# Corv/CUDA-GMM-MPI

Measured on NVIDIA H100. Metric: EM iterations/sec at N=10M D=24 K=64; E-step HBM GB/s vs roofline, higher is better.
Workload: dtype f32

## Files before the change

### cuda-gmm-mpi_b200/csrc/kernels_tc.cu

```cuda
#include <cuda.h>
#include <cudaTypedefs.h>
#include <cuda_fp16.h>
#if defined(__F16C__) && defined(__AVX__)
#include <immintrin.h>
#endif
#include <cuda_runtime.h>

#include <cfloat>
#include <cmath>
#include <cstdio>
#include <cstdlib>
#include <cstring>
#include <string>
#include <type_traits>
#include <vector>

#include "host_math.h"
#include "kernels_tc.cuh"
#include "mstep_rows.h"
#include "tc_ptx.cuh"

namespace gmm {

using namespace ptx;

#define TC_CUDA_TRY(expr)                                                                     \
    do {                                                                                      \
        cudaError_t e_ = (expr);                                                              \
        if (e_ != cudaSuccess)                                                                \
            return fail(GMM_ERR_CUDA, std::string(#expr) + ": " + cudaGetErrorString(e_));    \
    } while (0)

constexpr int kTE = 32;
constexpr int kNCL = 32;
constexpr int kNST = 3;
constexpr int kNRAW = 4;
constexpr int kChunkSub = 4;
constexpr int kChunkSub2 = 16;
constexpr int kPhiBits = 11;
constexpr float kGammaScale = 1024.0f;
constexpr float kGammaMagic = 1.5f * 134217728.0f;

template <int D, int NCL_> struct MCfg {
    static_assert(D % 4 == 0, "tensor M-step: D must be a multiple of 4");
    static_assert(NCL_ == 32 || NCL_ == 64, "tensor M-step: 32 or 64 clusters per CTA");
    static constexpr int NCL = NCL_;
    static constexpr int HPC = 64 / NCL;
    static constexpr int F = 1 + D + D * (D + 1) / 2;
    static constexpr int S = D / 4;
    static constexpr int MT = (4 * ((1 + 2 * S + S * (D / 2) + 7) / 8) * 8 + 127) / 128;
    static constexpr int G_PART = NCL * kTE * 2;
    static constexpr int G_STAGE = 3 * G_PART;
    static constexpr int RAWZ = (D * kTE * 4 + 1023) / 1024 * 1024;
    static constexpr int RAWX = RAWZ + 1024;
    static constexpr int RAWG = NCL * kTE * 4;
    static constexpr int OFF_G = 0;
    static constexpr int OFF_RAWX = OFF_G + kNST * G_STAGE;
    static constexpr int OFF_RAWG = OFF_RAWX + kNRAW * RAWX;
    static constexpr int NCT = MT * 128;
    static constexpr int OFF_RACC = OFF_RAWG + kNRAW * RAWG;
    static constexpr int OFF_BAR = OFF_RACC + 32 * NCT * 4;
    static constexpr int SMEM_BYTES = OFF_BAR + 512;
    static constexpr int THREADS = 128 + NCT;
    static constexpr int REG_LAUNCH = (65536 / THREADS) / 8 * 8 > 255 ? 255 : (65536 / THREADS) / 8 * 8;
    static constexpr int REG_P = MT == 1 ? REG_LAUNCH : 56;
    static constexpr int REG_C = MT == 3 ? 152 : (MT == 2 ? 224 : REG_LAUNCH);
    static_assert(128 * REG_P + NCT * REG_C <= THREADS * REG_LAUNCH, "register pools");
    static_assert(OFF_RAWX % 1024 == 0 && RAWX % 1024 == 0 && RAWZ % 1024 == 0, "SWIZZLE_128B TMA destinations need 1024-byte alignment");
    static_assert(OFF_RAWG % 1024 == 0 && RAWG % 1024 == 0, "SWIZZLE_128B TMA destinations need 1024-byte alignment");
    static_assert(MT <= 3, "feature tiles");
};

template <int R, int L>
__device__ __forceinline__ void set_regs() {
    if constexpr (R < L) asm volatile("setmaxnreg.dec.sync.aligned.u32 %0;" ::"n"(R));
    else if constexpr (R > L) asm volatile("setmaxnreg.inc.sync.aligned.u32 %0;" ::"n"(R));
}

struct MMagic { float lin, prod; };

__device__ __forceinline__ void tma_load_2d(void* smem_dst, const CUtensorMap* tmap, int c0, int c1, uint64_t* bar) {
    asm volatile(
        "cp.async.bulk.tensor.2d.shared::cluster.global.mbarrier::complete_tx::bytes [%0], [%1, {%2, %3}], [%4];"
        ::"r"(smem_u32(smem_dst)), "l"(reinterpret_cast<uint64_t>(tmap)), "r"(c0), "r"(c1), "r"(smem_u32(bar)) : "memory");
}

__device__ __forceinline__ float2 lds_f2(uint32_t addr) {
    float2 v;
    asm volatile("ld.shared.v2.f32 {%0, %1}, [%2];" : "=f"(v.x), "=f"(v.y) : "r"(addr) : "memory");
    return v;
}

__device__ __forceinline__ void feature_split(float a, float b, float m, float& h, float& l) {
    h = __fsub_rn(__fmaf_rn(a, b, m), m);
    l = __fmaf_rn(a, b, -h);
}

#ifndef GMM_MSTEP_CUT
#define GMM_MSTEP_CUT 0
#endif

__device__ __forceinline__ void build_half(const float2 (&za)[4], const float2 (&zb0)[4], const float2 (&zb1)[4], float m0, float m1,
                                           uint32_t (&hi)[2][4], uint32_t (&lo)[2][4]) {
#pragma unroll
    for (int p = 0; p < 4; p++) {
        const int ks = p >> 1, u = p & 1;
#if GMM_MSTEP_CUT == 2
        hi[ks][2 * u] = __float_as_uint(zb0[p].x); hi[ks][2 * u + 1] = __float_as_uint(zb1[p].x);
        lo[ks][2 * u] = __float_as_uint(zb0[p].y); lo[ks][2 * u + 1] = __float_as_uint(zb1[p].y);
        (void)za; (void)m0; (void)m1;
#else
        float h0, l0, h1, l1, h2, l2, h3, l3;
        feature_split(za[p].x, zb0[p].x, m0, h0, l0);
        feature_split(za[p].y, zb0[p].y, m0, h1, l1);
        feature_split(za[p].x, zb1[p].x, m1, h2, l2);
        feature_split(za[p].y, zb1[p].y, m1, h3, l3);
        hi[ks][2 * u] = pack_half2(h0, h1);
        hi[ks][2 * u + 1] = pack_half2(h2, h3);
        lo[ks][2 * u] = pack_half2(l0, l1);
        lo[ks][2 * u + 1] = pack_half2(l2, l3);
#endif
    }
}

__device__ __forceinline__ void load_row(uint32_t addr, float2 (&z)[4]) {
#pragma unroll
    for (int p = 0; p < 4; p++) z[p] = lds_f2(addr ^ (uint32_t)(p << 5));
}

template <int NCL>
__device__ __forceinline__ void issue_half(float (&ex)[NCL / 2], float (&rm)[NCL / 2], const uint32_t (&hi)[2][4], const uint32_t (&lo)[2][4],
                                           uint32_t gam, bool new1, bool new2) {
#pragma unroll
    for (int ks = 0; ks < kTE / 16; ks++) {
        const uint64_t hdesc = make_smem_desc(gam + ks * 256,  128,  512);
        const uint64_t ldesc = make_smem_desc(gam + NCL * kTE * 2 + ks * 256, 128, 512);
        const uint64_t sdesc = make_smem_desc(gam + 2 * NCL * kTE * 2 + ks * 256, 128, 512);
#if GMM_MSTEP_CUT == 1
        asm volatile("" ::"r"(hi[ks][0]), "r"(hi[ks][1]), "r"(hi[ks][2]), "r"(hi[ks][3]), "r"(lo[ks][0]), "r"(lo[ks][1]), "r"(lo[ks][2]),
                     "r"(lo[ks][3]), "l"(hdesc), "l"(ldesc), "l"(sdesc));
        (void)ex; (void)rm; (void)new1; (void)new2;
#else
        if constexpr (NCL == 32) {
            wgmma_m64n32k16_rs(ex, hi[ks][0], hi[ks][1], hi[ks][2], hi[ks][3], hdesc, ks > 0 || !new1);
            wgmma_m64n32k16_rs(rm, hi[ks][0], hi[ks][1], hi[ks][2], hi[ks][3], ldesc, ks > 0 || !new2);
            wgmma_m64n32k16_rs(rm, lo[ks][0], lo[ks][1], lo[ks][2], lo[ks][3], sdesc, true);
        } else {
            wgmma_m64n64k16_rs(ex, hi[ks][0], hi[ks][1], hi[ks][2], hi[ks][3], hdesc, ks > 0 || !new1);
            wgmma_m64n64k16_rs(rm, hi[ks][0], hi[ks][1], hi[ks][2], hi[ks][3], ldesc, ks > 0 || !new2);
            wgmma_m64n64k16_rs(rm, lo[ks][0], lo[ks][1], lo[ks][2], lo[ks][3], sdesc, true);
        }
#endif
    }
}

__device__ __forceinline__ bool chain_ends(int i, int mt, int nsub) { return ((i + mt) % kChunkSub) == kChunkSub - 1 || i == nsub - 1; }
__device__ __forceinline__ bool chain_starts(int i, int mt) { return i == 0 || ((i + mt) % kChunkSub) == 0; }
__device__ __forceinline__ bool chain2_ends(int i, int mt, int nsub) { return ((i + mt) % kChunkSub2) == kChunkSub2 - 1 || i == nsub - 1; }
__device__ __forceinline__ bool chain2_starts(int i, int mt) { return i == 0 || ((i + mt) % kChunkSub2) == 0; }

template <int D, int NCL, bool WT = false>
__global__ void __launch_bounds__(MCfg<D, NCL>::THREADS, 1)
mstep_tc_kernel(const __grid_constant__ CUtensorMap tm_x, const __grid_constant__ CUtensorMap tm_g, int n, int K,
                float* __restrict__ scratch, int events_per_cta, const __grid_constant__ MMagic magic, const int* __restrict__ opmap,
                const float* __restrict__ wts, float w_max, float w_inv) {
    using C = MCfg<D, NCL>;
    constexpr int HPC = C::HPC;
    extern __shared__ __align__(1024) uint8_t smem[];
    uint64_t* bars = reinterpret_cast<uint64_t*>(smem + C::OFF_BAR);
    uint64_t* raw_full = bars;
    uint64_t* raw_empty = bars + kNRAW;
    uint64_t* op_full = bars + 2 * kNRAW;
    uint64_t* op_empty = op_full + kNST;

    const int warp = threadIdx.x >> 5, lane = threadIdx.x & 31;
    const int range = blockIdx.x / (2 / HPC), part = blockIdx.x % (2 / HPC);
    const int e_begin = range * events_per_cta;
    const int e_end = min(n, e_begin + events_per_cta);
    const int nsub = (e_end - e_begin + kTE - 1) / kTE;
    const int k0 = blockIdx.y * NCL;

    for (int i = threadIdx.x; i < kNRAW * 256; i += C::THREADS)
        reinterpret_cast<float*>(smem + C::OFF_RAWX + (i >> 8) * C::RAWX + C::RAWZ)[i & 255] = 1.0f;
    if (threadIdx.x == 0) {
        for (int s = 0; s < kNRAW; s++) { mbar_init(&raw_full[s], 1); mbar_init(&raw_empty[s], 3 + 4 * C::MT); }
        for (int s = 0; s < kNST; s++) { mbar_init(&op_full[s], 3); mbar_init(&op_empty[s], 4 * C::MT); }
        fence_mbar_init();
    }
    __syncthreads();

    if (warp < 4) {
        set_regs<C::REG_P, C::REG_LAUNCH>();
        if (warp == 0) {
            const int nbox = min(NCL, K - k0 + kNCL - 1) / kNCL;
            if (elect_one()) {
                for (int i = 0; i < nsub; i++) {
                    const int st = i % kNRAW, ph = (i / kNRAW) & 1;
                    mbar_wait_parked(&raw_empty[st], ph ^ 1, 500);
                    mbar_arrive_expect_tx(&raw_full[st], kTE * D * 4 + nbox * kNCL * kTE * 4);
                    const int e0 = e_begin + i * kTE;
                    tma_load_2d(smem + C::OFF_RAWX + st * C::RAWX, &tm_x, e0, 0, &raw_full[st]);
                    for (int b = 0; b < nbox; b++)
                        tma_load_2d(smem + C::OFF_RAWG + st * C::RAWG + b * kNCL * kTE * 4, &tm_g, e0, k0 + b * kNCL, &raw_full[st]);
                }
            }
        } else {
            const int bt = threadIdx.x - 32;
            constexpr int NITEM = 4 * NCL, NIT = (NITEM + 95) / 96;
            for (int i = 0; i < nsub; i++) {
                const int rs = i % kNRAW, rph = (i / kNRAW) & 1;
                const int os = i % kNST, oph = (i / kNST) & 1;
                [[maybe_unused]] float wv[8];
                if constexpr (WT) {
                    const float4* wp = reinterpret_cast<const float4*>(wts + e_begin + i * kTE + 8 * ((bt & 31) >> 3));
                    const float4 wa = __ldg(wp), wb = __ldg(wp + 1);
                    wv[0] = wa.x; wv[1] = wa.y; wv[2] = wa.z; wv[3] = wa.w; wv[4] = wb.x; wv[5] = wb.y; wv[6] = wb.z; wv[7] = wb.w;
#pragma unroll
                    for (int v = 0; v < 8; v++) wv[v] = wv[v] == w_max ? 1.0f : __fmul_rn(wv[v], w_inv);
                }
                mbar_wait_parked(&raw_full[rs], rph, 200);
                mbar_wait_parked(&op_empty[os], oph ^ 1, 200);
                uint8_t* g_hi = smem + C::OFF_G + os * C::G_STAGE;
                float dep = 0.0f;
#pragma unroll
                for (int u = 0; u < NIT; u++) {
                    const int it = bt + 96 * u;
                    if (it >= NITEM) break;
                    const int kg = it >> 5, l = it & 31;
                    const int k = kg * 8 + (l & 7), ce = l >> 3;
                    const uint8_t* grow = smem + C::OFF_RAWG + rs * C::RAWG + k * (kTE * 4);
                    const float4 a = *reinterpret_cast<const float4*>(grow + (((2 * ce) ^ (k & 7)) << 4));
                    const float4 b = *reinterpret_cast<const float4*>(grow + (((2 * ce + 1) ^ (k & 7)) << 4));
                    float g[8] = {a.x, a.y, a.z, a.w, b.x, b.y, b.z, b.w};
                    dep += a.x + b.x;
                    if constexpr (WT) {
#pragma unroll
                        for (int v = 0; v < 8; v++) g[v] = __fmul_rn(g[v], wv[v]);
                    }
                    float hi[8], lo[8];
#pragma unroll
                    for (int v = 0; v < 8; v++) {
                        hi[v] = __fsub_rn(__fmaf_rn(g[v], kGammaScale, kGammaMagic), kGammaMagic);
                        lo[v] = __fmaf_rn(g[v], kGammaScale, -hi[v]);
                    }
                    *reinterpret_cast<uint4*>(g_hi + kg * 512 + l * 16) =
                        make_uint4(pack_half2(hi[0], hi[1]), pack_half2(hi[2], hi[3]), pack_half2(hi[4], hi[5]), pack_half2(hi[6], hi[7]));
                    *reinterpret_cast<uint4*>(g_hi + C::G_PART + kg * 512 + l * 16) =
                        make_uint4(pack_half2(lo[0], lo[1]), pack_half2(lo[2], lo[3]), pack_half2(lo[4], lo[5]), pack_half2(lo[6], lo[7]));
                    *reinterpret_cast<uint4*>(g_hi + 2 * C::G_PART + kg * 512 + l * 16) =
                        make_uint4(pack_half2(g[0] * kGammaScale, g[1] * kGammaScale), pack_half2(g[2] * kGammaScale, g[3] * kGammaScale),
                                   pack_half2(g[4] * kGammaScale, g[5] * kGammaScale), pack_half2(g[6] * kGammaScale, g[7] * kGammaScale));
                }
                __syncwarp();
                if (lane == 0) mbar_arrive_after(&raw_empty[rs], dep);
                else asm volatile("" ::"f"(dep));
                fence_proxy_async_smem();
                __syncwarp();
                if (lane == 0) mbar_arrive(&op_full[os]);
            }
        }
    } else {
        set_regs<C::REG_C, C::REG_LAUNCH>();
        const int cw = __shfl_sync(0xffffffffu, (warp - 4) >> 2, 0);
        const int hx = HPC == 2 ? 2 * cw : part * C::MT + cw;
        const int mt = hx >> 1;
        const int ct = threadIdx.x - 128;
        const int wq = warp & 3, gid = lane >> 2, qd = lane & 3;
        float* racc = reinterpret_cast<float*>(smem + C::OFF_RACC) + ct;
#pragma unroll
        for (int j = 0; j < 32; j++) racc[j * C::NCT] = 0.0f;
        constexpr int NSLOT = 2 * HPC;
        uint32_t fa, fb[NSLOT];
        float mg[NSLOT];
        {
            const int* om = opmap + hx * 64 + wq * 16 + gid;
            auto addr = [&](int code) {
                const uint32_t row = code >= kRowOne ? (uint32_t)(C::RAWZ / 128 + code - kRowOne) : (uint32_t)code;
                return row * 128 + ((((uint32_t)qd >> 1) ^ (row & 7)) << 4) + ((uint32_t)qd & 1) * 8;
            };
#pragma unroll
            for (int s = 0; s < NSLOT; s++) {
                const int c = om[(s >> 1) * 64 + (s & 1) * 8];
                const int a = c & 255, b = c >> 8;
                if (s == 0) fa = addr(a);
                fb[s] = addr(b);
                mg[s] = a >= kRowOne && b >= kRowOne ? 0.0f : (a >= kRowOne || b >= kRowOne ? magic.lin : magic.prod);
            }
        }
        const uint32_t zs0 = smem_u32(smem + C::OFF_RAWX);
        float ex[HPC][NCL / 2], rm[HPC][NCL / 2];
#pragma unroll
        for (int h = 0; h < HPC; h++)
#pragma unroll
            for (int j = 0; j < NCL / 2; j++) { ex[h][j] = 0.0f; rm[h][j] = 0.0f; }
        auto add_to_racc = [&](float (&acc)[HPC][NCL / 2]) {
#pragma unroll
            for (int c = 0; c < 2; c++) {
#pragma unroll
                for (int j = 0; j < 16; j++) {
                    const int q = 16 * c + j;
                    racc[q * C::NCT] += acc[q / (NCL / 2)][q % (NCL / 2)];
                }
                asm volatile("" ::: "memory");
            }
        };
        uint32_t fh[2][2][4], fl[2][2][4];
        float2 za[4];
        int held = -1;
        auto group = [&](int i, auto hc, uint32_t (&gh)[2][4], uint32_t (&gl)[2][4]) {
            constexpr int h = decltype(hc)::value;
            const int rs = i % kNRAW, rph = (i / kNRAW) & 1;
            const int os = i % kNST, oph = (i / kNST) & 1;
            const uint32_t zst = zs0 + rs * C::RAWX;
            const uint32_t gam = smem_u32(smem + C::OFF_G + os * C::G_STAGE);
            const bool new1 = chain_starts(i, mt), new2 = chain2_starts(i, mt);
            if constexpr (h == 0) {
                mbar_wait_parked(&raw_full[rs], rph, 100);
                load_row(zst + fa, za);
            }
            float2 zb0[4], zb1[4];
            load_row(zst + fb[2 * h], zb0);
            load_row(zst + fb[2 * h + 1], zb1);
            build_half(za, zb0, zb1, mg[2 * h], mg[2 * h + 1], gh, gl);
            if constexpr (h == 0) mbar_wait_parked(&op_full[os], oph, 100);
            wgmma_fence();
            issue_half<NCL>(ex[h], rm[h], gh, gl, gam, new1, new2);
            wgmma_commit();
            if constexpr (h == HPC - 1) {
                __syncwarp();
                if (lane == 0) mbar_arrive(&raw_empty[rs]);
            }
            wgmma_wait<1>();
            if constexpr (h == 0) {
                __syncwarp();
                if (lane == 0 && held >= 0) mbar_arrive(&op_empty[held]);
            }
            if constexpr (h == HPC - 1) {
                held = os;
                if (chain_ends(i, mt, nsub)) {
                    wgmma_wait<0>();
                    __syncwarp();
                    if (lane == 0) mbar_arrive(&op_empty[os]);
                    held = -1;
#if GMM_MSTEP_CUT != 3
                    add_to_racc(ex);
                    if (chain2_ends(i, mt, nsub)) add_to_racc(rm);
#endif
                }
            }
        };
        using H0 = std::integral_constant<int, 0>;
        using H1 = std::integral_constant<int, 1>;
        if constexpr (HPC == 2) {
            for (int i = 0; i < nsub; i++) {
                group(i, H0{}, fh[0], fl[0]);
                group(i, H1{}, fh[1], fl[1]);
            }
        } else {
            int i = 0;
            for (; i + 1 < nsub; i += 2) {
                group(i, H0{}, fh[0], fl[0]);
                group(i + 1, H0{}, fh[1], fl[1]);
            }
            if (i < nsub) group(i, H0{}, fh[0], fl[0]);
        }
        wgmma_wait<0>();
#if GMM_MSTEP_CUT == 3
#pragma unroll
        for (int h = 0; h < HPC; h++)
#pragma unroll
            for (int j = 0; j < NCL / 2; j++) ex[h][j] += rm[h][j];
        add_to_racc(ex);
#endif
        const int nranges = gridDim.x * HPC / 2;
#pragma unroll
        for (int h = 0; h < HPC; h++)
#pragma unroll
            for (int j = 0; j < NCL / 2; j += 2) {
                const int q = h * (NCL / 2) + j;
                const int row = ((hx & 1) + h) * 64 + wq * 16 + gid + 8 * ((j >> 1) & 1);
                const int col = (j >> 2) * 8 + 2 * qd;
                const int ty = blockIdx.y * (NCL / kNCL) + col / kNCL;
                float* dst = scratch + ((((size_t)ty * nranges + range) * C::MT + mt) * 128 + row) * kNCL + col % kNCL;
                *reinterpret_cast<float2*>(dst) = make_float2(racc[q * C::NCT], racc[(q + 1) * C::NCT]);
            }
    }
}

__global__ void standardise_soa_kernel(const float* __restrict__ xs, float* __restrict__ zs, size_t pitch, int n, int D,
                                       const float* __restrict__ shift_f, const float* __restrict__ inv_scale_f) {
    const int d = blockIdx.y;
    const float s = shift_f[d], isc = inv_scale_f[d];
    const float* x = xs + (size_t)d * pitch;
    float* z = zs + (size_t)d * pitch;
    for (long long e = (long long)blockIdx.x * blockDim.x + threadIdx.x; e < n; e += (long long)gridDim.x * blockDim.x)
        z[e] = __fmul_rn(__fsub_rn(x[e], s), isc);
}

__global__ void __launch_bounds__(256)
mstep_tc_finalize_kernel(const float* __restrict__ scratch, int ncta_x, int MT, int K, int F, const int3* __restrict__ rowmap,
                         const double* __restrict__ scale, double* __restrict__ stats, double wscale) {
    constexpr int NQ = 256 / kNCL;
    __shared__ double part[NQ][kNCL];
    const int3 rm = rowmap[blockIdx.x];
    if (rm.x < 0) return;
    const int mt = blockIdx.x / 128, row = blockIdx.x % 128;
    const int col = threadIdx.x & (kNCL - 1), q = threadIdx.x / kNCL;
    double fac = wscale / (double)kGammaScale;
    if (rm.y >= 0) fac *= scale[rm.y];
    if (rm.z >= 0) fac *= scale[rm.z];
    for (int ty = 0; ty * kNCL < K; ty++) {
        double s = 0;
        for (int cx = q; cx < ncta_x; cx += NQ)
            s += (double)scratch[(((size_t)(ty * ncta_x + cx) * MT + mt) * 128 + row) * kNCL + col];
        part[q][col] = s;
        __syncthreads();
        const int k = ty * kNCL + col;
        if (q == 0 && k < K) {
            double t = 0;
#pragma unroll
            for (int u = 0; u < NQ; u++) t += part[u][col];
            stats[(size_t)k * F + rm.x] += t * fac;
        }
        __syncthreads();
    }
}


template <int D> struct ECfg {
    static_assert(D % 8 == 0, "tensor E-step: D must be a multiple of 8");
    static constexpr int CP = D / 8;
    static constexpr int NLO = (CP + 1 + 1) / 2 * 2;
    static constexpr int NCHKB = CP + NLO;
    static constexpr int GB = 16;
    static constexpr int N = GB * 8;
    static constexpr int MAXSG = 64 / GB;
    static constexpr int B_BLOCK = NCHKB * N * 16;
    static constexpr int B_SG = CP * B_BLOCK;
    static constexpr int OFF_B = 0;
    static constexpr int OFF_CK = OFF_B + MAXSG * B_SG;
    static constexpr int OFF_SH = OFF_CK + 512;
    static constexpr int OFF_BAR = OFF_SH + 256;
    static constexpr int SMEM_BYTES = OFF_BAR + 64;
    static constexpr int NWG = 2;
    static constexpr int THREADS = 128 * NWG;
};

template <int D> struct EsCfg {
    using E = ECfg<D>;
    static constexpr bool SPLIT = D > 8;
    static constexpr int NMMA = 2;
    static constexpr int THREADS = SPLIT ? 128 * 2 * NMMA : E::THREADS;
    static constexpr int NSLOT = 3;
    static constexpr int SLOT = 64 * 64 * 4;
    static constexpr int OFF_SLOT = (E::SMEM_BYTES + 127) / 128 * 128;
    static constexpr int OFF_STAT = OFF_SLOT + NSLOT * SLOT;
    static constexpr int OFF_EBAR = OFF_STAT + NSLOT * 2 * 64 * 4;
    static constexpr int SMEM_BYTES = SPLIT ? OFF_EBAR + 4 * NSLOT * 8 : E::SMEM_BYTES;
    static constexpr int REG_LAUNCH = 65536 / (128 * 2 * NMMA) / 8 * 8;
    static constexpr int REG_MMA = 184;
    static constexpr int REG_EPI = 72;
    static_assert(128 * NMMA * (REG_MMA + REG_EPI) <= 128 * 2 * NMMA * REG_LAUNCH, "register pools");
    static_assert(SMEM_BYTES <= 232448, "shared memory budget");
};

__device__ __forceinline__ uint32_t slot_swz(int e) { return (uint32_t)(((e & 1) << 2 | (e & 2)) ^ ((e >> 2) & 7)); }

__device__ __forceinline__ void sts_f4(uint32_t addr, float a, float b, float c, float d) {
    asm volatile("st.shared.v4.f32 [%0], {%1, %2, %3, %4};" ::"r"(addr), "f"(a), "f"(b), "f"(c), "f"(d) : "memory");
}
__device__ __forceinline__ float4 lds_f4(uint32_t addr) {
    float4 v;
    asm volatile("ld.shared.v4.f32 {%0, %1, %2, %3}, [%4];" : "=f"(v.x), "=f"(v.y), "=f"(v.z), "=f"(v.w) : "r"(addr) : "memory");
    return v;
}
__device__ __forceinline__ void epi_bar(int id) { asm volatile("bar.sync %0, 128;" ::"r"(id) : "memory"); }

#ifndef GMM_ESTEP_CUT
#define GMM_ESTEP_CUT 0
#endif

template <int D>
__device__ __forceinline__ void tc_stage_operand(uint8_t* smem, const uint8_t* __restrict__ b_img, const float* __restrict__ ck,
                                                 const float* __restrict__ shift_f, const float* __restrict__ inv_scale_f, int NSG) {
    using C = ECfg<D>;
    uint64_t* b_full = reinterpret_cast<uint64_t*>(smem + C::OFF_BAR);
    float* ck_s = reinterpret_cast<float*>(smem + C::OFF_CK);
    float* sh_s = reinterpret_cast<float*>(smem + C::OFF_SH);
    if (threadIdx.x == 0) { mbar_init(b_full, 1); fence_mbar_init(); }
    if (threadIdx.x < 64) { ck_s[threadIdx.x] = ck[threadIdx.x] * 1.4426950408889634f; ck_s[64 + threadIdx.x] = ck[64 + threadIdx.x]; }
    if (threadIdx.x < D) { sh_s[threadIdx.x] = shift_f[threadIdx.x]; sh_s[32 + threadIdx.x] = inv_scale_f[threadIdx.x]; }
    __syncthreads();
    if (threadIdx.x == 0) {
        mbar_arrive_expect_tx(b_full, (uint32_t)NSG * C::B_SG);
        for (int g = 0; g < NSG * C::CP; g++) tma_load_1d(smem + C::OFF_B + g * C::B_BLOCK, b_img + (size_t)g * C::B_BLOCK, C::B_BLOCK, b_full);
    }
}

template <int D>
__device__ __forceinline__ void tc_split_rows(const float2 (&xa)[D / 8], const float2 (&xb)[D / 8], const float* sh_s, const float* isc_s,
                                              int qd, uint32_t (&zh)[D / 8][2], uint32_t (&zl)[D / 8][2]) {
#pragma unroll
    for (int j = 0; j < D / 8; j++) {
        const float s0 = sh_s[8 * j + 2 * qd], s1 = sh_s[8 * j + 2 * qd + 1];
        const float i0 = isc_s[8 * j + 2 * qd], i1 = isc_s[8 * j + 2 * qd + 1];
#pragma unroll
        for (int r = 0; r < 2; r++) {
            const float2 x = r ? xb[j] : xa[j];
            const float z0 = __fmul_rn(__fsub_rn(x.x, s0), i0), z1 = __fmul_rn(__fsub_rn(x.y, s1), i1);
            const __half2 h = __floats2half2_rn(z0, z1);
            const float2 f = __half22float2(h);
            zh[j][r] = *reinterpret_cast<const uint32_t*>(&h);
            zl[j][r] = pack_half2(z0 - f.x, z1 - f.y);
        }
    }
}

template <int D>
__device__ __forceinline__ void tc_issue_group(float (&acc)[32], const uint32_t (&zh)[D / 8][2], const uint32_t (&zl)[D / 8][2],
                                               uint32_t bsg, int c, int h, uint32_t ones) {
    using C = ECfg<D>;
    constexpr int CP = C::CP;
    constexpr uint32_t CH = C::N * 16;
    const uint32_t bb = bsg + (uint32_t)c * C::B_BLOCK + (uint32_t)h * (CH / 2);
    wgmma_fence();
#pragma unroll
    for (int j = c; j < CP; j++)
        wgmma_m64n64k16_rs(acc, zh[j][0], zh[j][1], zh[j][0], zh[j][1], make_smem_desc(bb + j * CH, CP * CH, 128), j > c);
#pragma unroll
    for (int p = c; p < CP + 1; p += 2) {
        const int x = p, y = p + 1;
        if (y <= CP) {
            const uint32_t yc = y < CP ? (uint32_t)y : 2u * CP;
            const uint32_t a2 = y < CP ? zl[y < CP ? y : 0][0] : ones, a3 = y < CP ? zl[y < CP ? y : 0][1] : ones;
            wgmma_m64n64k16_rs(acc, zl[x][0], zl[x][1], a2, a3, make_smem_desc(bb + x * CH, (yc - x) * CH, 128), true);
        } else {
            wgmma_m64n64k16_rs(acc, 0u, 0u, ones, ones, make_smem_desc(bb + c * CH, (2 * CP - c) * CH, 128), true);
        }
    }
}

template <int D, int NSG>
__device__ __forceinline__ void tc_tile_logits(const uint32_t (&zh)[D / 8][2], const uint32_t (&zl)[D / 8][2], uint32_t bsm,
                                               const float* ck_s, int qd, uint32_t ones, float (&lg)[ECfg<D>::MAXSG][8]) {
    using C = ECfg<D>;
    constexpr int CP = C::CP;
    float acc[2][32];
    tc_issue_group<D>(acc[0], zh, zl, bsm, 0, 0, ones);
    wgmma_commit();
#pragma unroll
    for (int sg = 0; sg < C::MAXSG; sg++) {
        if (sg >= NSG) {
#pragma unroll
            for (int u = 0; u < 8; u++) lg[sg][u] = -INFINITY;
            continue;
        }
        const uint32_t bsg = bsm + (uint32_t)sg * C::B_SG;
        float sq[32];
#pragma unroll
        for (int u = 0; u < 32; u++) sq[u] = 0.f;
#pragma unroll
        for (int c = 0; c < CP; c++) {
#pragma unroll
            for (int h = 0; h < 2; h++) {
                if (sg + 1 == NSG && c + 1 == CP && h == 1) {
                    wgmma_wait<0>();
                } else {
                    if (h == 0) tc_issue_group<D>(acc[1], zh, zl, bsg, c, 1, ones);
                    else if (c + 1 < CP) tc_issue_group<D>(acc[0], zh, zl, bsg, c + 1, 0, ones);
                    else tc_issue_group<D>(acc[0], zh, zl, bsg + C::B_SG, 0, 0, ones);
                    wgmma_commit();
                    wgmma_wait<1>();
                }
                wgmma_pin(acc[h]);
                const float(&a)[32] = acc[h];
#if GMM_ESTEP_CUT == 1
                sq[0] += a[0];
#else
#pragma unroll
                for (int i = 0; i < 8; i++) {
                    float& s0 = sq[16 * h + 2 * i];
                    float& s1 = sq[16 * h + 2 * i + 1];
                    s0 = fmaf(a[4 * i], a[4 * i], fmaf(a[4 * i + 1], a[4 * i + 1], s0));
                    s1 = fmaf(a[4 * i + 2], a[4 * i + 2], fmaf(a[4 * i + 3], a[4 * i + 3], s1));
                }
#endif
            }
        }
#if GMM_ESTEP_CUT == 1
        for (int u = 0; u < 8; u++) lg[sg][u] = sq[0];
        continue;
#endif
        float w[16];
        const bool b1 = qd & 1, b2 = (qd >> 1) & 1;
#pragma unroll
        for (int u = 0; u < 16; u++) {
            const float send = b1 ? sq[u] : sq[16 + u], keep = b1 ? sq[16 + u] : sq[u];
            w[u] = keep + __shfl_xor_sync(0xffffffffu, send, 1);
        }
#pragma unroll
        for (int u = 0; u < 8; u++) {
            const float send = b2 ? w[u] : w[8 + u], keep = b2 ? w[8 + u] : w[u];
            const float qv = keep + __shfl_xor_sync(0xffffffffu, send, 2);
            const int k = sg * C::GB + 8 * (qd & 1) + 4 * (qd >> 1) + (u >> 1);
            lg[sg][u] = fmaf(ck_s[64 + k], qv, ck_s[k]);
        }
    }
}

template <int D, int NSG>
__device__ __forceinline__ void estep_tile_logits(const uint32_t (&zh)[D / 8][2], const uint32_t (&zl)[D / 8][2], uint32_t bsm,
                                                  const float* ck_s, int qd, uint32_t ones, uint32_t slot, int r0, float& cut_sum) {
    using C = ECfg<D>;
    constexpr int CP = C::CP, NG = NSG * CP * 2;
    float acc[2][32];
    tc_issue_group<D>(acc[0], zh, zl, bsm, 0, 0, ones);
    wgmma_commit();
    const uint32_t cq = 2 * (qd & 1) + (qd >> 1);
    const uint32_t row0 = slot + (uint32_t)r0 * 256, row1 = row0 + 8 * 256;
    const uint32_t sw0 = slot_swz(r0), sw1 = slot_swz(r0 + 8);
    float sq[32];
#pragma unroll
    for (int g = 0; g < NG; g++) {
        const int sg = g / (2 * CP), c = (g / 2) % CP, h = g & 1;
        if (c == 0 && h == 0) {
#pragma unroll
            for (int u = 0; u < 32; u++) sq[u] = 0.f;
        }
        if (g + 1 < NG) {
            const int gn = g + 1;
            tc_issue_group<D>(acc[gn & 1], zh, zl, bsm + (uint32_t)(gn / (2 * CP)) * C::B_SG, (gn / 2) % CP, gn & 1, ones);
            wgmma_commit();
            wgmma_wait<1>();
// ... 1269 lines not shown
```

Measured before the change: 140.4.

## Split M-step raw TMA ring into separate x and gamma rings with deeper stages

The single raw-input ring, which coupled the x tile and the gamma tiles under one barrier pair, is split into independent z (x) and g (gamma) rings, each with its own full/empty mbarriers and stage count. Gamma buffers are now released by the conversion warps alone, and x buffers by the consumer warps alone. The stage depths become per-config constants: 6/6/4 for 64 clusters per CTA, and 4/4/3 otherwise. This decouples producer stalls and deepens prefetch, at the cost of more shared memory, which a new static_assert checks against the budget. A debug cut switch (GMM_MSTEP_CUT==4) is also added for the conversion loop.

```diff
diff --git a/cuda-gmm-mpi_b200/csrc/kernels_tc.cu b/cuda-gmm-mpi_b200/csrc/kernels_tc.cu
--- a/cuda-gmm-mpi_b200/csrc/kernels_tc.cu
+++ b/cuda-gmm-mpi_b200/csrc/kernels_tc.cu
@@ -33,14 +33,21 @@
 
 constexpr int kTE = 32;
 constexpr int kNCL = 32;
-constexpr int kNST = 3;
-constexpr int kNRAW = 4;
 constexpr int kChunkSub = 4;
 constexpr int kChunkSub2 = 16;
 constexpr int kPhiBits = 11;
 constexpr float kGammaScale = 1024.0f;
 constexpr float kGammaMagic = 1.5f * 134217728.0f;
 
+#ifndef GMM_MSTEP_NZ
+#define GMM_MSTEP_NZ 0
+#endif
+#ifndef GMM_MSTEP_NG
+#define GMM_MSTEP_NG 0
+#endif
+#ifndef GMM_MSTEP_NST
+#define GMM_MSTEP_NST 0
+#endif
 template <int D, int NCL_> struct MCfg {
     static_assert(D % 4 == 0, "tensor M-step: D must be a multiple of 4");
     static_assert(NCL_ == 32 || NCL_ == 64, "tensor M-step: 32 or 64 clusters per CTA");
@@ -54,13 +61,16 @@
     static constexpr int RAWZ = (D * kTE * 4 + 1023) / 1024 * 1024;
     static constexpr int RAWX = RAWZ + 1024;
     static constexpr int RAWG = NCL * kTE * 4;
+    static constexpr int NZ = GMM_MSTEP_NZ > 0 ? GMM_MSTEP_NZ : (NCL == 64 ? 6 : 4);
+    static constexpr int NG = GMM_MSTEP_NG > 0 ? GMM_MSTEP_NG : (NCL == 64 ? 6 : 4);
+    static constexpr int NST = GMM_MSTEP_NST > 0 ? GMM_MSTEP_NST : (NCL == 64 ? 4 : 3);
     static constexpr int OFF_G = 0;
-    static constexpr int OFF_RAWX = OFF_G + kNST * G_STAGE;
-    static constexpr int OFF_RAWG = OFF_RAWX + kNRAW * RAWX;
+    static constexpr int OFF_RAWX = OFF_G + NST * G_STAGE;
+    static constexpr int OFF_RAWG = OFF_RAWX + NZ * RAWX;
     static constexpr int NCT = MT * 128;
-    static constexpr int OFF_RACC = OFF_RAWG + kNRAW * RAWG;
+    static constexpr int OFF_RACC = OFF_RAWG + NG * RAWG;
     static constexpr int OFF_BAR = OFF_RACC + 32 * NCT * 4;
-    static constexpr int SMEM_BYTES = OFF_BAR + 512;
+    static constexpr int SMEM_BYTES = OFF_BAR + 2 * (NZ + NG + NST) * 8;
     static constexpr int THREADS = 128 + NCT;
     static constexpr int REG_LAUNCH = (65536 / THREADS) / 8 * 8 > 255 ? 255 : (65536 / THREADS) / 8 * 8;
     static constexpr int REG_P = MT == 1 ? REG_LAUNCH : 56;
@@ -69,6 +79,7 @@
     static_assert(OFF_RAWX % 1024 == 0 && RAWX % 1024 == 0 && RAWZ % 1024 == 0, "SWIZZLE_128B TMA destinations need 1024-byte alignment");
     static_assert(OFF_RAWG % 1024 == 0 && RAWG % 1024 == 0, "SWIZZLE_128B TMA destinations need 1024-byte alignment");
     static_assert(MT <= 3, "feature tiles");
+    static_assert(SMEM_BYTES <= 232448, "shared memory budget");
 };
 
 template <int R, int L>
@@ -167,11 +178,14 @@
     using C = MCfg<D, NCL>;
     constexpr int HPC = C::HPC;
     extern __shared__ __align__(1024) uint8_t smem[];
+    constexpr int NZ = C::NZ, NG = C::NG, NST = C::NST;
     uint64_t* bars = reinterpret_cast<uint64_t*>(smem + C::OFF_BAR);
-    uint64_t* raw_full = bars;
-    uint64_t* raw_empty = bars + kNRAW;
-    uint64_t* op_full = bars + 2 * kNRAW;
-    uint64_t* op_empty = op_full + kNST;
+    uint64_t* z_full = bars;
+    uint64_t* z_empty = z_full + NZ;
+    uint64_t* g_full = z_empty + NZ;
+    uint64_t* g_empty = g_full + NG;
+    uint64_t* op_full = g_empty + NG;
+    uint64_t* op_empty = op_full + NST;
 
     const int warp = threadIdx.x >> 5, lane = threadIdx.x & 31;
     const int range = blockIdx.x / (2 / HPC), part = blockIdx.x % (2 / HPC);
@@ -180,11 +194,12 @@
     const int nsub = (e_end - e_begin + kTE - 1) / kTE;
     const int k0 = blockIdx.y * NCL;
 
-    for (int i = threadIdx.x; i < kNRAW * 256; i += C::THREADS)
+    for (int i = threadIdx.x; i < NZ * 256; i += C::THREADS)
         reinterpret_cast<float*>(smem + C::OFF_RAWX + (i >> 8) * C::RAWX + C::RAWZ)[i & 255] = 1.0f;
     if (threadIdx.x == 0) {
-        for (int s = 0; s < kNRAW; s++) { mbar_init(&raw_full[s], 1); mbar_init(&raw_empty[s], 3 + 4 * C::MT); }
-        for (int s = 0; s < kNST; s++) { mbar_init(&op_full[s], 3); mbar_init(&op_empty[s], 4 * C::MT); }
+        for (int s = 0; s < NZ; s++) { mbar_init(&z_full[s], 1); mbar_init(&z_empty[s], 4 * C::MT); }
+        for (int s = 0; s < NG; s++) { mbar_init(&g_full[s], 1); mbar_init(&g_empty[s], 3); }
+        for (int s = 0; s < NST; s++) { mbar_init(&op_full[s], 3); mbar_init(&op_empty[s], 4 * C::MT); }
         fence_mbar_init();
     }
     __syncthreads();
@@ -195,21 +210,24 @@
             const int nbox = min(NCL, K - k0 + kNCL - 1) / kNCL;
             if (elect_one()) {
                 for (int i = 0; i < nsub; i++) {
-                    const int st = i % kNRAW, ph = (i / kNRAW) & 1;
-                    mbar_wait_parked(&raw_empty[st], ph ^ 1, 500);
-                    mbar_arrive_expect_tx(&raw_full[st], kTE * D * 4 + nbox * kNCL * kTE * 4);
                     const int e0 = e_begin + i * kTE;
-                    tma_load_2d(smem + C::OFF_RAWX + st * C::RAWX, &tm_x, e0, 0, &raw_full[st]);
+                    const int gs = i % NG, gph = (i / NG) & 1;
+                    mbar_wait_parked(&g_empty[gs], gph ^ 1, 500);
+                    mbar_arrive_expect_tx(&g_full[gs], nbox * kNCL * kTE * 4);
                     for (int b = 0; b < nbox; b++)
-                        tma_load_2d(smem + C::OFF_RAWG + st * C::RAWG + b * kNCL * kTE * 4, &tm_g, e0, k0 + b * kNCL, &raw_full[st]);
+                        tma_load_2d(smem + C::OFF_RAWG + gs * C::RAWG + b * kNCL * kTE * 4, &tm_g, e0, k0 + b * kNCL, &g_full[gs]);
+                    const int zs = i % NZ, zph = (i / NZ) & 1;
+                    mbar_wait_parked(&z_empty[zs], zph ^ 1, 500);
+                    mbar_arrive_expect_tx(&z_full[zs], kTE * D * 4);
+                    tma_load_2d(smem + C::OFF_RAWX + zs * C::RAWX, &tm_x, e0, 0, &z_full[zs]);
                 }
             }
         } else {
             const int bt = threadIdx.x - 32;
             constexpr int NITEM = 4 * NCL, NIT = (NITEM + 95) / 96;
             for (int i = 0; i < nsub; i++) {
-                const int rs = i % kNRAW, rph = (i / kNRAW) & 1;
-                const int os = i % kNST, oph = (i / kNST) & 1;
+                const int gs = i % NG, gph = (i / NG) & 1;
+                const int os = i % NST, oph = (i / NST) & 1;
                 [[maybe_unused]] float wv[8];
                 if constexpr (WT) {
                     const float4* wp = reinterpret_cast<const float4*>(wts + e_begin + i * kTE + 8 * ((bt & 31) >> 3));
@@ -218,17 +236,17 @@
 #pragma unroll
                     for (int v = 0; v < 8; v++) wv[v] = wv[v] == w_max ? 1.0f : __fmul_rn(wv[v], w_inv);
                 }
-                mbar_wait_parked(&raw_full[rs], rph, 200);
+                mbar_wait_parked(&g_full[gs], gph, 200);
                 mbar_wait_parked(&op_empty[os], oph ^ 1, 200);
                 uint8_t* g_hi = smem + C::OFF_G + os * C::G_STAGE;
                 float dep = 0.0f;
 #pragma unroll
-                for (int u = 0; u < NIT; u++) {
+                for (int u = 0; u < (GMM_MSTEP_CUT == 4 ? 0 : NIT); u++) {
                     const int it = bt + 96 * u;
                     if (it >= NITEM) break;
                     const int kg = it >> 5, l = it & 31;
                     const int k = kg * 8 + (l & 7), ce = l >> 3;
-                    const uint8_t* grow = smem + C::OFF_RAWG + rs * C::RAWG + k * (kTE * 4);
+                    const uint8_t* grow = smem + C::OFF_RAWG + gs * C::RAWG + k * (kTE * 4);
                     const float4 a = *reinterpret_cast<const float4*>(grow + (((2 * ce) ^ (k & 7)) << 4));
                     const float4 b = *reinterpret_cast<const float4*>(grow + (((2 * ce + 1) ^ (k & 7)) << 4));
                     float g[8] = {a.x, a.y, a.z, a.w, b.x, b.y, b.z, b.w};
@@ -252,7 +270,7 @@
                                    pack_half2(g[4] * kGammaScale, g[5] * kGammaScale), pack_half2(g[6] * kGammaScale, g[7] * kGammaScale));
                 }
                 __syncwarp();
-                if (lane == 0) mbar_arrive_after(&raw_empty[rs], dep);
+                if (lane == 0) mbar_arrive_after(&g_empty[gs], dep);
                 else asm volatile("" ::"f"(dep));
                 fence_proxy_async_smem();
                 __syncwarp();
@@ -309,13 +327,13 @@
         int held = -1;
         auto group = [&](int i, auto hc, uint32_t (&gh)[2][4], uint32_t (&gl)[2][4]) {
             constexpr int h = decltype(hc)::value;
-            const int rs = i % kNRAW, rph = (i / kNRAW) & 1;
-            const int os = i % kNST, oph = (i / kNST) & 1;
-            const uint32_t zst = zs0 + rs * C::RAWX;
+            const int zs = i % NZ, zph = (i / NZ) & 1;
+            const int os = i % NST, oph = (i / NST) & 1;
+            const uint32_t zst = zs0 + zs * C::RAWX;
             const uint32_t gam = smem_u32(smem + C::OFF_G + os * C::G_STAGE);
             const bool new1 = chain_starts(i, mt), new2 = chain2_starts(i, mt);
             if constexpr (h == 0) {
-                mbar_wait_parked(&raw_full[rs], rph, 100);
+                mbar_wait_parked(&z_full[zs], zph, 100);
                 load_row(zst + fa, za);
             }
             float2 zb0[4], zb1[4];
@@ -328,7 +346,7 @@
             wgmma_commit();
             if constexpr (h == HPC - 1) {
                 __syncwarp();
-                if (lane == 0) mbar_arrive(&raw_empty[rs]);
+                if (lane == 0) mbar_arrive(&z_empty[zs]);
             }
             wgmma_wait<1>();
             if constexpr (h == 0) {
```

New measurement: 142.8 (median of 6 runs). 1.7% higher.
